# lucidrains/audiolm-pytorch

Hardware: AMD Instinct MI355X
Metric: audio-tokens/sec fwd+bwd, CoarseTransformer d=1024 seq=2048 (higher is better)
Workload: dtype bf16

## Files before the change

audiolm-pytorch_amd/csrc/gemm.hip:

```cpp
#include <algorithm>
#include <cstdlib>
#include <type_traits>

#include "common.hpp"
#include "../../include/audiolm_hip.h"

#ifndef ALM_GEMM_AUX_A
#define ALM_GEMM_AUX_A 0
#endif
#ifndef ALM_GEMM_AUX_B
#define ALM_GEMM_AUX_B 0
#endif

namespace {

constexpr int BK = 64;
constexpr unsigned OOB = 0x80000000u;

typedef __attribute__((address_space(3))) void lds_void;

struct GemmParams {
    const bf16_t* A;
    const bf16_t* B;
    void* C;
// ... 17 lines not shown
    int inl_slices = 0;
};

__device__ __forceinline__ int grouped_tile(int bid, int tiles_m, int tiles_n, int g) {
    const bool rows = g > 0;
    const int ga = rows ? g : -g;
    const int t_in = rows ? tiles_n : tiles_m, t_gr = rows ? tiles_m : tiles_n;
    const int per_group = ga * t_in;
    const int group = bid / per_group, rem = bid % per_group;
    const int first = group * ga;
    const int gsz = min(t_gr - first, ga);
    const int a = first + rem % gsz, b = rem / gsz;
    return rows ? (a | (b << 16)) : (b | (a << 16));
}

template <int BM, int BN, int WM, int WN, int TM, int TNB, bool OUT_F32>
__device__ __forceinline__ void gemm_epilogue(const GemmParams& p, f32x16 (&acc)[TM][TNB], unsigned char* slabs, long long coff0, int m0, int n0,
                                              int wave, int wr, int wc, int lane, int lr, int lh) {
    {
        constexpr int ES = OUT_F32 ? 4 : 2;
        constexpr int WCOLS = 32 * TNB;
        constexpr int ROWB = WCOLS * ES;
        constexpr int NCH = ROWB / 16;
        constexpr int SLAB = 32 * ROWB;
        unsigned char* Cb = reinterpret_cast<unsigned char*>(p.C) + coff0 * ES;
        const bool fast = !p.accumulate && ((p.ldc * ES) & 15) == 0 && ((uintptr_t)Cb & 15) == 0 && (p.N % (16 / ES)) == 0;
        if (fast) {
            unsigned char* slab = slabs + wave * SLAB;
            const int ncol0 = n0 + wc * (BN / WN);
#pragma unroll
            for (int i = 0; i < TM; ++i) {
                const int mrow0 = m0 + wr * (BM / WM) + i * 32;
#pragma unroll
                for (int j = 0; j < TNB; ++j)
#pragma unroll
                    for (int g = 0; g < 4; ++g) {
                        const int c0 = j * 32 + 8 * g + 4 * lh;
                        float v[4];
#pragma unroll
                        for (int c = 0; c < 4; ++c) {
                            v[c] = acc[i][j][4 * g + c] * p.alpha;
                            if (p.bias && ncol0 + c0 + c < p.N) v[c] += p.bias[ncol0 + c0 + c];
                        }
                        if (OUT_F32) {
                            const int ch = c0 / 4;
                            *reinterpret_cast<float4*>(slab + lr * ROWB + ((ch ^ (lr & (NCH - 1))) << 4)) = make_float4(v[0], v[1], v[2], v[3]);
                        } else {
                            const int ch = c0 / 8;
                            *reinterpret_cast<uint2*>(slab + lr * ROWB + ((ch ^ (lr & (NCH - 1))) << 4) + lh * 8) =
                                make_uint2(pack_bf2(v[0], v[1]), pack_bf2(v[2], v[3]));
                        }
                    }
                constexpr int LPR = NCH;
                constexpr int RPI = 64 / LPR;
#pragma unroll
                for (int it = 0; it < 32 / RPI; ++it) {
                    const int row = it * RPI + lane / LPR, ch = lane % LPR;
                    const uint4 val = *reinterpret_cast<const uint4*>(slab + row * ROWB + ((ch ^ (row & (NCH - 1))) << 4));
                    const int gm = mrow0 + row, gn = ncol0 + ch * (16 / ES);
#if defined(ALM_GEMM_WHATIF_NOSTORE)
                    if (gm < p.M && gn < p.N && val.x == 0x7fc12345u) *reinterpret_cast<uint4*>(Cb + ((long long)gm * p.ldc + gn) * ES) = val;
#else
                    if (gm < p.M && gn < p.N) {
                        uint4* dst = reinterpret_cast<uint4*>(Cb + ((long long)gm * p.ldc + gn) * ES);
                        typedef unsigned int u32x4 __attribute__((ext_vector_type(4)));
                        if (p.nt_store) __builtin_nontemporal_store(u32x4{val.x, val.y, val.z, val.w}, reinterpret_cast<u32x4*>(dst)); else *dst = val;
                    }
#endif
                }
            }
            return;
        }
    }
    const long long coff = coff0;
    const bool vec_ok = OUT_F32 ? ((p.ldc & 3) == 0 && (coff & 3) == 0 && ((uintptr_t)p.C & 15) == 0)
                                : ((p.ldc & 3) == 0 && (coff & 3) == 0 && ((uintptr_t)p.C & 7) == 0);
#pragma unroll
    for (int i = 0; i < TM; ++i) {
        const int gm = m0 + wr * (BM / WM) + i * 32 + lr;
        if (gm >= p.M) continue;
#pragma unroll
        for (int j = 0; j < TNB; ++j) {
#pragma unroll
            for (int g = 0; g < 4; ++g) {
                const int gn = n0 + wc * (BN / WN) + j * 32 + 8 * g + 4 * lh;
                if (gn >= p.N) continue;
                float v[4];
#pragma unroll
                for (int c = 0; c < 4; ++c) {
                    v[c] = acc[i][j][4 * g + c] * p.alpha;
                    if (p.bias && gn + c < p.N) v[c] += p.bias[gn + c];
                }
                const long long idx = coff + (long long)gm * p.ldc + gn;
                if (OUT_F32) {
                    float* C = reinterpret_cast<float*>(p.C) + idx;
                    if (vec_ok && gn + 3 < p.N) {
                        float4 o = make_float4(v[0], v[1], v[2], v[3]);
                        if (p.accumulate) { const float4 w = *reinterpret_cast<const float4*>(C); o.x += w.x; o.y += w.y; o.z += w.z; o.w += w.w; }
                        *reinterpret_cast<float4*>(C) = o;
                    } else {
#pragma unroll
                        for (int c = 0; c < 4; ++c)
                            if (gn + c < p.N) C[c] = p.accumulate ? C[c] + v[c] : v[c];
                    }
                } else {
                    bf16_t* C = reinterpret_cast<bf16_t*>(p.C) + idx;
                    if (vec_ok && gn + 3 < p.N) {
                        if (p.accumulate) {
                            const uint2 w = *reinterpret_cast<const uint2*>(C);
                            v[0] += __uint_as_float(w.x << 16); v[1] += __uint_as_float(w.x & 0xffff0000u);
                            v[2] += __uint_as_float(w.y << 16); v[3] += __uint_as_float(w.y & 0xffff0000u);
                        }
                        *reinterpret_cast<uint2*>(C) = make_uint2(pack_bf2(v[0], v[1]), pack_bf2(v[2], v[3]));
                    } else {
#pragma unroll
                        for (int c = 0; c < 4; ++c)
                            if (gn + c < p.N) C[c] = f2bf(p.accumulate ? bf2f(C[c]) + v[c] : v[c]);
                    }
                }
            }
        }
    }
}

template <int N>
__device__ __forceinline__ void wait_vmcnt() {
    static_assert(N == 0 || N == 8 || N == 16, "add the literal");
    if constexpr (N == 0) asm volatile("s_waitcnt vmcnt(0)" ::: "memory");
    else if constexpr (N == 8) asm volatile("s_waitcnt vmcnt(8)" ::: "memory");
    else asm volatile("s_waitcnt vmcnt(16)" ::: "memory");
}

template <int BM, int BN, int WM, int WN, bool TNMODE, bool OUT_F32, int NS = 2>
// ... 197 lines not shown
#pragma unroll 1
        for (int kt = 0; kt < nk; ++kt) {
            const int newer = min(nk - 1 - kt, NS - 2);
            if (newer >= 2) wait_vmcnt<16>(); else if (newer == 1) wait_vmcnt<8>(); else wait_vmcnt<0>();
            asm volatile("s_waitcnt lgkmcnt(0)" ::: "memory");
            __builtin_amdgcn_s_barrier();
            __builtin_amdgcn_sched_barrier(0);
            kstep(smem + ((kt + NS - 1) % NS) * STAGE, smem + (kt % NS) * STAGE, kt);
        }
        __syncthreads();
    }

    constexpr int ES = OUT_F32 ? 4 : 2;
    static_assert(NW * 32 * (32 * TNB * ES) <= 2 * STAGE, "epilogue slab");
    const long long coff0 = z1 * p.sC1 + z2 * p.sC2 + (p.ksplit > 0 ? zs * p.sCk : 0);
    gemm_epilogue<BM, BN, WM, WN, TM, TNB, OUT_F32>(p, acc, smem, coff0, m0, n0, wave, wr, wc, lane, lr, lh);
}

template <int BM, int BN, int WM, int WN, bool TNMODE, bool OUT_F32>
__global__ __launch_bounds__(WM * WN * 64) void gemm_kernel(GemmParams p) {
    gemm_body<BM, BN, WM, WN, TNMODE, OUT_F32>(p, blockIdx.x, blockIdx.y, blockIdx.z);
}

template <int BM, int BN, int WM, int WN, bool TNMODE, bool OUT_F32, int NS>
__global__ __launch_bounds__(WM * WN * 64) void gemm_ring_kernel(GemmParams p) {
    gemm_body<BM, BN, WM, WN, TNMODE, OUT_F32, NS>(p, blockIdx.x, blockIdx.y, blockIdx.z);
}

template <int BM, int BN, int WM, int WN, bool TNMODE, bool OUT_F32>
__global__ __launch_bounds__(WM * WN * 64) void gemm_group2_kernel(GemmParams p0, GemmParams p1, int tiles0) {
    const bool second = (int)blockIdx.x >= tiles0;
    const GemmParams& p = second ? p1 : p0;
    gemm_body<BM, BN, WM, WN, TNMODE, OUT_F32>(p, second ? (int)blockIdx.x - tiles0 : (int)blockIdx.x, 0, 0);
}

#ifdef ALM_GEMM_PROBE
__device__ unsigned long long g_gemm_probe[16384 * 8];
#define GPROBE_DECL unsigned long long pacc[8] = {0, 0, 0, 0, 0, 0, 0, 0}; unsigned long long plast = __builtin_readcyclecounter();
#define GPROBE_T(i) do { __builtin_amdgcn_sched_barrier(0); const unsigned long long pt_ = __builtin_readcyclecounter(); __builtin_amdgcn_sched_barrier(0); pacc[i] += pt_ - plast; plast = pt_; } while (0)
#define GPROBE_FLUSH(slot) do { if (lane == 0 && (slot) < 16384) for (int i_ = 0; i_ < 8; ++i_) g_gemm_probe[(slot) * 8 + i_] = pacc[i_]; } while (0)
#else
#define GPROBE_DECL
#define GPROBE_T(i)
#define GPROBE_FLUSH(slot)
#endif

template <bool TNMODE, bool OUT_F32, bool INL = false>
__device__ __forceinline__ void gemm_stag_body(const GemmParams& p, const int bx, const int by, const int bz) {
    extern __shared__ __attribute__((aligned(1024))) unsigned char smem[];
    GPROBE_DECL
    constexpr int BM = 256, BN = 256, WM = 2, WN = 4, NW = 8, TM = 4, TNB = 2;
    constexpr int AH_BYTES = 128 * BK * 2, B_BYTES = BN * BK * 2;
    constexpr int B_BASE = 4 * AH_BYTES;
    static_assert(B_BASE + 3 * B_BYTES == 163840, "LDS map");

    const int tiles_m = (p.M + BM - 1) / BM, tiles_n = (p.N + BN - 1) / BN;
    int tm, tn, zb, zs;
    if (p.raster >= 1) {
        const int L = bx, xcd = L & 7, j = L >> 3;
        const bool m_major = tiles_m >= tiles_n;
        const int tmaj = m_major ? tiles_m : tiles_n, Q = m_major ? tiles_n : tiles_m;
        const int P = p.plimit > 0 ? p.plimit : tmaj * (p.nbt > 0 ? p.nbt : p.nb2);
// ... 53 lines not shown
#pragma unroll
    for (int j = 0; j < 4; ++j) {
        const int qa = j * 4 + wc;
        const int qb = wr * 16 + j * 4 + wc;
        dstA[j] = (unsigned)(qa * 1024);
        dstB[j] = (unsigned)(qb * 1024);
        if (!TNMODE) {
            const int rowa = wr * 128 + qa * 8 + (lane >> 3), rowb = qb * 8 + (lane >> 3);
            const int ca = (lane & 7) ^ ((rowa >> 1) & 7), cb = (lane & 7) ^ ((rowb >> 1) & 7);
            offA[j] = (unsigned)(rowa * p.lda * 2 + ca * 16);
            offB[j] = (unsigned)(rowb * p.ldb * 2 + cb * 16);
            kcA[j] = ca * 8;
            kcB[j] = cb * 8;
        } else {
            const int st = lane >> 3, kin = (lane >> 1) & 3, half = lane & 1;
            const int ka = qa * 4 + kin, ia = wr * 128 + st * 16 + half * 8;
            const int kgb = qb / 2, partb = qb % 2;
            const int kb = kgb * 4 + kin, ib = partb * 128 + st * 16 + half * 8;
            offA[j] = (unsigned)(ka * p.lda * 2 + ia * 2);
            offB[j] = (unsigned)(kb * p.ldb * 2 + ib * 2);
            kcA[j] = ka;
            kcB[j] = kb;
        }
    }
    const unsigned kstepA = TNMODE ? (unsigned)(BK * p.lda * 2) : (unsigned)(BK * 2);
    const unsigned kstepB = TNMODE ? (unsigned)(BK * p.ldb * 2) : (unsigned)(BK * 2);
    unsigned char* const myA = smem + wr * 2 * AH_BYTES;

    auto stage = [&](int j, unsigned char* ad, unsigned char* bd) {
        const int kleft = Krem - j * BK;
#pragma unroll
        for (int i = 0; i < 4; ++i) {
            const unsigned vo = (kcA[i] < kleft) ? offA[i] : OOB;
            __builtin_amdgcn_raw_ptr_buffer_load_lds(rsA, (lds_void*)(ad + dstA[i]), 16, vo, j * kstepA, 0, ALM_GEMM_AUX_A);
        }
#pragma unroll
        for (int i = 0; i < 4; ++i) {
            const unsigned vo = (kcB[i] < kleft) ? offB[i] : OOB;
            __builtin_amdgcn_raw_ptr_buffer_load_lds(rsB, (lds_void*)(bd + dstB[i]), 16, vo, j * kstepB, 0, ALM_GEMM_AUX_B);
        }
    };

    unsigned fragA[TM], fragB[TNB];
    if (!TNMODE) {
#pragma unroll
        for (int i = 0; i < TM; ++i) fragA[i] = (unsigned)((i * 32 + lr) * 128);
#pragma unroll
        for (int j = 0; j < TNB; ++j) fragB[j] = (unsigned)((wc * 64 + j * 32 + lr) * 128);
    } else {
        const int g = lane >> 4, s = lane & 15;
#pragma unroll
        for (int i = 0; i < TM; ++i) fragA[i] = (unsigned)((((g >> 1) * 2) * 8 + (i * 32) / 16 + (g & 1)) * 128 + s * 8);
#pragma unroll
        for (int j = 0; j < TNB; ++j) fragB[j] = (unsigned)((((g >> 1) * 2) * 16 + (wc * 64 + j * 32) / 16 + (g & 1)) * 128 + s * 8);
    }
    const unsigned sw = (unsigned)((lr >> 1) & 7);

    f32x16 acc[TM][TNB];
#pragma unroll
    for (int i = 0; i < TM; ++i)
#pragma unroll
        for (int j = 0; j < TNB; ++j)
#pragma unroll
            for (int r = 0; r < 16; ++r) acc[i][j][r] = 0.f;

    auto load_frags = [&](const unsigned char* sa, const unsigned char* sb, int ks, bf16x8 (&a)[TM], bf16x8 (&b)[TNB]) {
        if (!TNMODE) {
            const unsigned co = (((unsigned)(ks * 2 + lh)) ^ sw) << 4;
#pragma unroll
            for (int i = 0; i < TM; ++i) a[i] = *reinterpret_cast<const bf16x8*>(sa + fragA[i] + co);
#pragma unroll
            for (int j = 0; j < TNB; ++j) b[j] = *reinterpret_cast<const bf16x8*>(sb + fragB[j] + co);
        } else {
#pragma unroll
            for (int i = 0; i < TM; ++i) {
                const unsigned char* ad = sa + fragA[i] + ks * 4 * 8 * 128;
                a[i] = __builtin_shufflevector(lds_tr16(ad), lds_tr16(ad + 8 * 128), 0, 1, 2, 3, 4, 5, 6, 7);
            }
#pragma unroll
            for (int j = 0; j < TNB; ++j) {
                const unsigned char* bd = sb + fragB[j] + ks * 4 * 16 * 128;
                b[j] = __builtin_shufflevector(lds_tr16(bd), lds_tr16(bd + 16 * 128), 0, 1, 2, 3, 4, 5, 6, 7);
            }
        }
    };
    auto mfma_all = [&](const bf16x8 (&a)[TM], const bf16x8 (&b)[TNB]) {
#pragma unroll
        for (int i = 0; i < TM; ++i)
#pragma unroll
            for (int j = 0; j < TNB; ++j) acc[i][j] = __builtin_amdgcn_mfma_f32_32x32x16_bf16(b[j], a[i], acc[i][j], 0, 0, 0);
    };
    constexpr int NRD = (TNMODE ? 2 : 1) * (TM + TNB);
    auto compute = [&](const unsigned char* sa, const unsigned char* sb) {
        bf16x8 a0[TM], b0[TNB], a1[TM], b1[TNB];
        load_frags(sa, sb, 0, a0, b0);
        load_frags(sa, sb, 1, a1, b1);
        mfma_all(a0, b0);
        load_frags(sa, sb, 2, a0, b0);
        mfma_all(a1, b1);
        load_frags(sa, sb, 3, a1, b1);
        mfma_all(a0, b0);
        mfma_all(a1, b1);
        __builtin_amdgcn_sched_group_barrier(0x100, 2 * NRD, 0);
        for (int g = 0; g < 2; ++g) {
#pragma unroll
            for (int q = 0; q < TM * TNB; ++q) {
                __builtin_amdgcn_sched_group_barrier(0x008, 1, 0);
                if (q < NRD) __builtin_amdgcn_sched_group_barrier(0x100, 1, 0);
            }
            if (NRD > TM * TNB) __builtin_amdgcn_sched_group_barrier(0x100, NRD - TM * TNB, 0);
        }
        __builtin_amdgcn_sched_group_barrier(0x008, 2 * TM * TNB, 0);
    };

    const int nk = (Krem + BK - 1) / BK;
    auto Abuf = [&](int j) { return myA + (j & 1) * AH_BYTES; };
    auto Bbuf = [&](int j) { return smem + B_BASE + (j % 3) * B_BYTES; };
    auto pair = [&](unsigned char* __restrict__ dA, unsigned char* __restrict__ dB, const unsigned char* __restrict__ rA,
                    const unsigned char* __restrict__ rB, int i) {
        if (i < nk) stage(i, dA, dB);
        GPROBE_T(1);
        __builtin_amdgcn_s_barrier();
        GPROBE_T(2);
        if (i >= 1) compute(rA, rB);
        GPROBE_T(3);
        __syncthreads();
        GPROBE_T(4);
    };
    GPROBE_T(0);
    if (wr == 1) __syncthreads();
#pragma unroll 1
    for (int i = 0; i <= nk; ++i) pair(Abuf(i), Bbuf(i), Abuf(i + 1), Bbuf(i + 2), i);
    if (wr == 0) __syncthreads();
    __builtin_amdgcn_s_barrier();

    if constexpr (INL) {
        typedef unsigned int u32x4 __attribute__((ext_vector_type(4)));
        constexpr int SLAB_BYTES = BM * BN * 4, NCHUNK = TM * TNB * 4;
        const int S = p.inl_slices;
        const int tile_lin = zb * (tiles_m * tiles_n) + tm * tiles_n + tn;
        unsigned char* const slab0 = reinterpret_cast<unsigned char*>(p.inl_ws) + (long long)tile_lin * S * SLAB_BYTES;
        {
            const auto rs = __builtin_amdgcn_make_buffer_rsrc(slab0 + (long long)zs * SLAB_BYTES, 0, SLAB_BYTES, 0x00020000);
#pragma unroll
            for (int i = 0; i < TM; ++i)
#pragma unroll
                for (int j = 0; j < TNB; ++j)
#pragma unroll
                    for (int g = 0; g < 4; ++g) {
                        const u32x4 v = {__float_as_uint(acc[i][j][4 * g]), __float_as_uint(acc[i][j][4 * g + 1]), __float_as_uint(acc[i][j][4 * g + 2]),
                                         __float_as_uint(acc[i][j][4 * g + 3])};
                        __builtin_amdgcn_raw_buffer_store_b128(v, rs, t * 16, ((i * TNB + j) * 4 + g) * 8192, 16);
                    }
        }
        asm volatile("s_waitcnt vmcnt(0)" ::: "memory");
        __syncthreads();
        unsigned* const flag = reinterpret_cast<unsigned*>(smem + 163840 - 16);
        if (t == 0) {
            const unsigned old = __hip_atomic_fetch_add(p.inl_cnt + tile_lin, 1u, __ATOMIC_RELAXED, __HIP_MEMORY_SCOPE_AGENT);
            const unsigned last = old == (unsigned)(S - 1);
            if (last) __hip_atomic_store(p.inl_cnt + tile_lin, 0u, __ATOMIC_RELAXED, __HIP_MEMORY_SCOPE_AGENT);
            *flag = last;
        }
        __syncthreads();
        if (*flag == 0) return;
        auto add_slab = [&](int sl, auto first_c) {
            constexpr bool FIRST = decltype(first_c)::value;
            const auto rs = __builtin_amdgcn_make_buffer_rsrc(slab0 + (long long)sl * SLAB_BYTES, 0, SLAB_BYTES, 0x00020000);
#pragma unroll
            for (int cb = 0; cb < NCHUNK; cb += 4) {
                u32x4 v[4];
#pragma unroll
                for (int c = 0; c < 4; ++c) v[c] = __builtin_amdgcn_raw_buffer_load_b128(rs, t * 16, (cb + c) * 8192, 16);
#pragma unroll
                for (int c = 0; c < 4; ++c)
#pragma unroll
                    for (int e = 0; e < 4; ++e) {
                        const int ai = (cb + c) / (4 * TNB), aj = ((cb + c) / 4) % TNB, ar = 4 * ((cb + c) % 4) + e;
                        acc[ai][aj][ar] = FIRST ? __uint_as_float(v[c][e]) : acc[ai][aj][ar] + __uint_as_float(v[c][e]);
                    }
            }
        };
        if (S == 2) {
            add_slab(1 - zs, std::false_type{});
        } else {
            add_slab(0, std::true_type{});
#pragma unroll 1
            for (int sl = 1; sl < S; ++sl) add_slab(sl, std::false_type{});
        }
    }

    const long long coff0 = z1 * p.sC1 + z2 * p.sC2 + (p.ksplit > 0 ? zs * p.sCk : 0);
    GPROBE_T(5);
    gemm_epilogue<BM, BN, WM, WN, TM, TNB, OUT_F32>(p, acc, smem, coff0, m0, n0, wave, wr, wc, lane, lr, lh);
    GPROBE_T(6);
    GPROBE_FLUSH((bx + gridDim.x * (by + gridDim.y * bz)) * 8 + wave);
}


template <bool TNMODE, bool OUT_F32>
__global__ __launch_bounds__(512) void gemm_stag_kernel(GemmParams p) {
    gemm_stag_body<TNMODE, OUT_F32>(p, blockIdx.x, blockIdx.y, blockIdx.z);
}

template <bool OUT_F32>
__global__ __launch_bounds__(512) void gemm_stag_inl_kernel(GemmParams p) {
    gemm_stag_body<false, OUT_F32, true>(p, blockIdx.x, blockIdx.y, blockIdx.z);
}

template <bool TNMODE, bool OUT_F32>
__global__ __launch_bounds__(512) void gemm_stag_group2_kernel(GemmParams p0, GemmParams p1, int tiles0) {
    const bool second = (int)blockIdx.x >= tiles0;
    const GemmParams& p = second ? p1 : p0;
    gemm_stag_body<TNMODE, OUT_F32>(p, second ? (int)blockIdx.x - tiles0 : (int)blockIdx.x, 0, 0);
}

template <bool TNMODE, bool OUT_F32>
__global__ __launch_bounds__(256) void gemm_w4_kernel(GemmParams p) {
    extern __shared__ __attribute__((aligned(1024))) unsigned char smem[];
    GPROBE_DECL
    constexpr int BM = 256, BN = 256, WM = 2, WN = 2, NW = 4, TM = 4, TNB = 4;
    constexpr int A_BYTES = BM * BK * 2, B_BYTES = BN * BK * 2, STAGE = A_BYTES + B_BYTES;
    constexpr int NIA = BM / 8 / NW, NIB = BN / 8 / NW;
    static_assert(NIA + NIB == 16, "the counted waits below assume 16 pieces per wave and stage");

    const int tiles_m = (p.M + BM - 1) / BM, tiles_n = (p.N + BN - 1) / BN;
    int tm, tn, zb, zs;
    if (p.raster >= 1) {
        const int L = blockIdx.x, xcd = L & 7, j = L >> 3;
// ... 214 lines not shown
        __builtin_amdgcn_sched_barrier(0);
        GPROBE_T(4);
    };
    using T = std::true_type;
    using F = std::false_type;
    int kt = 0;
#pragma unroll 1
    for (; kt + 2 < nk; ++kt) kstep(smem + (kt & 1) * STAGE, smem + ((kt & 1) ^ 1) * STAGE, kt, T{}, T{});
    if (kt + 1 < nk) { kstep(smem + (kt & 1) * STAGE, smem + ((kt & 1) ^ 1) * STAGE, kt, F{}, T{}); ++kt; }
    kstep(smem + (kt & 1) * STAGE, smem + ((kt & 1) ^ 1) * STAGE, kt, F{}, F{});
    __syncthreads();

    constexpr int ES = OUT_F32 ? 4 : 2;
    static_assert(NW * 32 * (32 * TNB * ES) <= 2 * STAGE, "epilogue slab");
    const long long coff0 = z1 * p.sC1 + z2 * p.sC2 + (p.ksplit > 0 ? zs * p.sCk : 0);
    gemm_epilogue<BM, BN, WM, WN, TM, TNB, OUT_F32>(p, acc, smem, coff0, m0, n0, wave, wr, wc, lane, lr, lh);
    GPROBE_T(6);
    GPROBE_FLUSH((blockIdx.x + gridDim.x * (blockIdx.y + gridDim.y * blockIdx.z)) * 4 + wave);
}

__global__ __launch_bounds__(256) void splitk_reduce_kernel(const float* __restrict__ ws, int splits, long long mn, long long slice_stride, int N,
                                                            float* __restrict__ C, long long ldc, long long sC, int accumulate,
                                                            int nb2 = 0x40000000, long long sC1 = 0) {
    ws += (long long)blockIdx.y * mn;
    C += (long long)(blockIdx.y / nb2) * sC1 + (long long)(blockIdx.y % nb2) * sC;
    const bool vec = (N & 3) == 0 && (ldc & 3) == 0 && ((uintptr_t)C & 15) == 0 && (mn & 3) == 0 && (slice_stride & 3) == 0;
    if (vec) {
        const long long mn4 = mn >> 2;
        for (long long i = (long long)blockIdx.x * 256 + threadIdx.x; i < mn4; i += (long long)gridDim.x * 256) {
            float4 s = make_float4(0.f, 0.f, 0.f, 0.f);
            for (int z = 0; z < splits; ++z) {
// ... 218 lines not shown

template <bool OUT_F32>
int launch_ring(const GemmParams& p, int ny, int nz, hipStream_t st) {
    constexpr int smem = 4 * (128 + 128) * BK * 2;
    static bool attr_done = false;
    auto kfn = gemm_ring_kernel<128, 128, 2, 2, false, OUT_F32, 4>;
    if (!attr_done) {
        hipError_t e = hipFuncSetAttribute(reinterpret_cast<const void*>(kfn), hipFuncAttributeMaxDynamicSharedMemorySize, smem);
        if (e != hipSuccess) return (int)e;
        attr_done = true;
    }
    hipLaunchKernelGGL(kfn, dim3(((p.M + 127) / 128) * ((p.N + 127) / 128), ny, nz), dim3(256), smem, st, p);
    return 0;
}

template <bool TNMODE, bool OUT_F32>
int launch_stag(const GemmParams& p, int ny, int nz, hipStream_t st) {
    constexpr int smem = 163840;
    static bool attr_done = false;
    auto kfn = gemm_stag_kernel<TNMODE, OUT_F32>;
    if (!attr_done) {
        hipError_t e = hipFuncSetAttribute(reinterpret_cast<const void*>(kfn), hipFuncAttributeMaxDynamicSharedMemorySize, smem);
        if (e != hipSuccess) return (int)e;
        attr_done = true;
    }
    const int tiles_m = (p.M + 255) / 256, tiles_n = (p.N + 255) / 256;
    if (p.raster >= 1) {
        const int tmaj = tiles_m >= tiles_n ? tiles_m : tiles_n, Q = tiles_m >= tiles_n ? tiles_n : tiles_m;
        const int PL = ((p.plimit > 0 ? p.plimit : tmaj * ny) + 7) / 8;
        hipLaunchKernelGGL(kfn, dim3(8 * PL * Q * nz), dim3(512), smem, st, p);
        return 0;
    }
    hipLaunchKernelGGL(kfn, dim3(tiles_m * tiles_n, ny, nz), dim3(512), smem, st, p);
    return 0;
}


template <bool OUT_F32>
int launch_stag_inl(const GemmParams& p, int ny, hipStream_t st) {
    constexpr int smem = 163840;
    static bool attr_done = false;
    auto kfn = gemm_stag_inl_kernel<OUT_F32>;
    if (!attr_done) {
        hipError_t e = hipFuncSetAttribute(reinterpret_cast<const void*>(kfn), hipFuncAttributeMaxDynamicSharedMemorySize, smem);
        if (e != hipSuccess) return (int)e;
        attr_done = true;
    }
    const int tiles_m = (p.M + 255) / 256, tiles_n = (p.N + 255) / 256;
    hipLaunchKernelGGL(kfn, dim3(tiles_m * tiles_n, ny, p.inl_slices), dim3(512), smem, st, p);
    return 0;
}

template <bool TNMODE, bool OUT_F32>
int launch_w4(const GemmParams& p, int ny, int nz, hipStream_t st) {
    constexpr int smem = 131072;
    static bool attr_done = false;
    auto kfn = gemm_w4_kernel<TNMODE, OUT_F32>;
// ... 41 lines not shown
template <bool TNMODE>
int launch_gemm(const GemmParams& p0, int ny, int nz, int out_f32, int tile, hipStream_t st, bool hook = true, bool only256 = false) {
    static const int big_tile = [] { const char* e = getenv("ALM_GEMM_BIG_TILE"); return e ? atoi(e) : 0; }();
    static const int nt_store = [] { const char* e = getenv("ALM_GEMM_NT_STORE"); return e ? atoi(e) : 0; }();
    GemmParams p = p0;
    int tl = pick_tile(p.M, p.N, ny * nz, tile, TNMODE);
    if (tl < 0) return ALM_ERR_UNSUPPORTED;
    p.group_m = pick_group(p, tl);
    p.nt_store = (nt_store == 1 || (nt_store == 2 && !out_f32)) ? 1 : 0;
    if (hook && tl != 1 && (big_tile == 2 || big_tile == 13 || big_tile == 14 || (big_tile == 11 && !only256))) tl = big_tile;
    static const int w4_mink = [] { const char* e = getenv("ALM_GEMM_W4_MINK"); return e ? atoi(e) : 0; }();
    if (hook && w4_mink > 0 && tl == 13 && tile == 0 && (p.ksplit > 0 ? p.ksplit : p.K) >= w4_mink) tl = 14;
    static const int w4_tn_mink = [] { const char* e = getenv("ALM_GEMM_W4_TN_MINK"); return e ? atoi(e) : 8192; }();
    if (TNMODE && hook && w4_tn_mink > 0 && tl == 13 && (p.ksplit > 0 ? p.ksplit : p.K) >= w4_tn_mink) tl = 14;
    if (tl == 14) return out_f32 ? launch_w4<TNMODE, true>(p, ny, nz, st) : launch_w4<TNMODE, false>(p, ny, nz, st);
    if (tl == 13) return out_f32 ? launch_stag<TNMODE, true>(p, ny, nz, st) : launch_stag<TNMODE, false>(p, ny, nz, st);
    static const int mid_tile = [] { const char* e = getenv("ALM_GEMM_MID_TILE"); return e ? atoi(e) : 0; }();
    if (!TNMODE && hook && mid_tile && tl == 1 && tile == 0 && p.ksplit == 0 && p.M >= 256 && p.N >= 512 &&
        (long long)((p.M + 255) / 256) * ((p.N + 127) / 128) * ny >= 192) tl = 15;
    static const int ring_on = [] { const char* e = getenv("ALM_GEMM_RING"); return e ? atoi(e) : 1; }();
    if (!TNMODE && hook && ring_on && tl == 1 && tile == 0 && p.ksplit == 0 && p.raster == 0 && p.K >= 256 &&
        (long long)((p.M + 127) / 128) * ((p.N + 127) / 128) * ny * nz <= 256) tl = 16;
    if (tl == 16) { if (TNMODE || p.raster != 0) return ALM_ERR_UNSUPPORTED; return out_f32 ? launch_ring<true>(p, ny, nz, st) : launch_ring<false>(p, ny, nz, st); }
    if (tl == 15) return out_f32 ? launch_cfg<256, 128, 4, 2, TNMODE, true>(p, ny, nz, st) : launch_cfg<256, 128, 4, 2, TNMODE, false>(p, ny, nz, st);
    if (tl == 11) return out_f32 ? launch_cfg<384, 256, 2, 4, TNMODE, true>(p, ny, nz, st) : launch_cfg<384, 256, 2, 4, TNMODE, false>(p, ny, nz, st);
    if (tl == 17) { if (TNMODE) return ALM_ERR_UNSUPPORTED; return out_f32 ? launch_cfg<320, 256, 2, 4, false, true>(p, ny, nz, st) : launch_cfg<320, 256, 2, 4, false, false>(p, ny, nz, st); }
    if (tl == 2) return out_f32 ? launch_cfg<256, 256, 2, 4, TNMODE, true>(p, ny, nz, st) : launch_cfg<256, 256, 2, 4, TNMODE, false>(p, ny, nz, st);
    return out_f32 ? launch_cfg<128, 128, 2, 2, TNMODE, true>(p, ny, nz, st) : launch_cfg<128, 128, 2, 2, TNMODE, false>(p, ny, nz, st);
}

bool view_too_big(long long rows, long long ld) { return rows * ld * 2 >= 0x7fffffffLL; }
// ... 35 lines not shown
    if (pl.slices == 1) return launch_gemm<false>(p0, ny, 1, out_f32, 13, st, false);
    const long long need = INL_CNT_BYTES + tiles * pl.slices * INL_SLAB_BYTES;
    if (!ws || ws_bytes < need || ((uintptr_t)ws & 15)) {
        if (force_slices > 0) return ALM_ERR_BAD_ARG;
        return launch_gemm<false>(p0, ny, 1, out_f32, 0, st);
    }
    GemmParams p = p0;
    const int ksteps = (p.K + BK - 1) / BK;
    p.ksplit = (ksteps + pl.slices - 1) / pl.slices * BK;
    p.sCk = 0;
    p.inl_slices = (p.K + p.ksplit - 1) / p.ksplit;
    if (p.inl_slices < 2) return launch_gemm<false>(p0, ny, 1, out_f32, 13, st, false);
    p.inl_cnt = reinterpret_cast<unsigned*>(ws);
    p.inl_ws = reinterpret_cast<float*>(reinterpret_cast<unsigned char*>(ws) + INL_CNT_BYTES);
    p.group_m = pick_group(p, 13);
    return out_f32 ? launch_stag_inl<true>(p, ny, st) : launch_stag_inl<false>(p, ny, st);
}

struct SplitPlan { int tile, slices; };

int pick_raster(int M, int N, int nb, int tile) {
    const int bm = tile >= 2 ? 256 : 128;
    const int tmm = (M + bm - 1) / bm, tnn = (N + bm - 1) / bm;
    const int P = (tmm >= tnn ? tmm : tnn) * nb;
    return (P % 8 == 0 || P >= 20) ? 1 : 0;
}
SplitPlan splitk_plan(int M, int N, int K, int nb) {
    SplitPlan best{1, 1};
    double best_t = 1e30;
    for (int tile = 1; tile <= 2; ++tile) {
        if (tile == 2 && (M < 256 || N < 256)) continue;
// ... 131 lines not shown
        const long long a = (long long)((M0 + 255) / 256) * ((N0 + 255) / 256), b = (long long)((M1 + 255) / 256) * ((N1 + 255) / 256);
        if (a + b >= 192 && a + b <= 256 && (a & 7) == 0) t0 = t1 = 13;
    }
    const int bm = t0 == 1 ? 128 : 256;
    const int tiles0 = ((M0 + bm - 1) / bm) * ((N0 + bm - 1) / bm), tiles1 = ((M1 + bm - 1) / bm) * ((N1 + bm - 1) / bm);
    if (!on || t0 != t1 || (t0 != 1 && t0 != 13) || (tiles0 & 7)) {
        int rc = alm_gemm_bf16_nt(A0, B0, C0, nullptr, M0, N0, K0, lda0, ldb0, ldc0, 1, 1, 0, 0, 0, 0, 0, 0, 1.f, out_f32, 0, stream);
        if (rc) return rc;
        return alm_gemm_bf16_nt(A1, B1, C1, nullptr, M1, N1, K1, lda1, ldb1, ldc1, 1, 1, 0, 0, 0, 0, 0, 0, 1.f, out_f32, 0, stream);
    }
    GemmParams p0{(const bf16_t*)A0, (const bf16_t*)B0, C0, nullptr, M0, N0, K0, lda0, ldb0, ldc0, 1, 0, 0, 0, 0, 0, 0, 1.f, 0, 0, 0, 0, 1};
    GemmParams p1{(const bf16_t*)A1, (const bf16_t*)B1, C1, nullptr, M1, N1, K1, lda1, ldb1, ldc1, 1, 0, 0, 0, 0, 0, 0, 1.f, 0, 0, 0, 0, 1};
    p0.group_m = pick_group(p0, t0);
    p1.group_m = pick_group(p1, t1);
    auto launch = [&](auto kfn, int which, int threads, int smem) -> int {
        static bool attr_done[4] = {false, false, false, false};
        if (!attr_done[which]) {
            hipError_t e = hipFuncSetAttribute(reinterpret_cast<const void*>(kfn), hipFuncAttributeMaxDynamicSharedMemorySize, smem);
            if (e != hipSuccess) return (int)e;
            attr_done[which] = true;
        }
        hipLaunchKernelGGL(kfn, dim3(tiles0 + tiles1), dim3(threads), smem, st, p0, p1, tiles0);
        return 0;
    };
    int rc;
    if (t0 == 1) rc = out_f32 ? launch(gemm_group2_kernel<128, 128, 2, 2, false, true>, 0, 256, 2 * (128 + 128) * BK * 2)
                              : launch(gemm_group2_kernel<128, 128, 2, 2, false, false>, 1, 256, 2 * (128 + 128) * BK * 2);
    else rc = out_f32 ? launch(gemm_stag_group2_kernel<false, true>, 2, 512, 163840) : launch(gemm_stag_group2_kernel<false, false>, 3, 512, 163840);
    if (rc) return rc;
    ALM_LAUNCH_CHECK();
    return 0;
}

extern "C" int alm_gemm_bf16_nt_tile(const void* A, const void* B, void* C, const float* bias, int M, int N, int K, long long lda,
                                     long long ldb, long long ldc, float alpha, int out_f32, int accumulate, int tile, void* stream) {
    if (M <= 0 || N <= 0) return 0;
    if (K <= 0 || (K & 7) || (lda & 7) || (ldb & 7) || ((uintptr_t)A & 15) || ((uintptr_t)B & 15)) return ALM_ERR_BAD_ARG;
    if (view_too_big(384, lda) || view_too_big(256, ldb)) return ALM_ERR_UNSUPPORTED;
    GemmParams p{(const bf16_t*)A, (const bf16_t*)B, C, bias, M, N, K, lda, ldb, ldc, 1, 0, 0, 0, 0, 0, 0, alpha, accumulate, 0, 0, 0, 1};
    int rc = launch_gemm<false>(p, 1, 1, out_f32, tile, (hipStream_t)stream, false);
    if (rc) return rc;
    ALM_LAUNCH_CHECK();
    return 0;
// ... 234 lines not shown
```

Before: 1.438 million.

## Use 16x16x32 MFMA in staggered 256-tile GEMM kernel by default

Adds an MF16 variant of the staggered 256x256 GEMM body that computes with 16x16x32 bf16 MFMA instructions instead of 32x32x16. This changes the fragment addressing, LDS swizzle and accumulator layout, and generalises the epilogue and inline split-K reduction to both accumulator shapes. The variant is on by default through an environment switch. The aim is a better MFMA issue and LDS-read interleaving schedule. The trade-off is more LDS fragment reads per MFMA and a riskier scheduling pattern.

```diff
diff --git a/audiolm-pytorch_amd/csrc/gemm.hip b/audiolm-pytorch_amd/csrc/gemm.hip
--- a/audiolm-pytorch_amd/csrc/gemm.hip
+++ b/audiolm-pytorch_amd/csrc/gemm.hip
@@ -55,9 +55,26 @@
     return rows ? (a | (b << 16)) : (b | (a << 16));
 }
 
-template <int BM, int BN, int WM, int WN, int TM, int TNB, bool OUT_F32>
-__device__ __forceinline__ void gemm_epilogue(const GemmParams& p, f32x16 (&acc)[TM][TNB], unsigned char* slabs, long long coff0, int m0, int n0,
-                                              int wave, int wr, int wc, int lane, int lr, int lh) {
+template <int TNB, typename AccV, int AM, int AN>
+__device__ __forceinline__ void acc_quad(AccV (&acc)[AM][AN], int i, int q, int lane, int& r, int& c0, float (&v)[4]) {
+    if constexpr (std::is_same<AccV, f32x16>::value) {
+        const int j = q / 4, g = q % 4;
+        r = lane & 31;
+        c0 = j * 32 + 8 * g + 4 * (lane >> 5);
+#pragma unroll
+        for (int c = 0; c < 4; ++c) v[c] = acc[i][j][4 * g + c];
+    } else {
+        const int h = q / (2 * TNB), j = q % (2 * TNB);
+        r = h * 16 + (lane & 15);
+        c0 = j * 16 + 4 * (lane >> 4);
+#pragma unroll
+        for (int c = 0; c < 4; ++c) v[c] = acc[2 * i + h][j][c];
+    }
+}
+
+template <int BM, int BN, int WM, int WN, int TM, int TNB, bool OUT_F32, typename AccV, int AM, int AN>
+__device__ __forceinline__ void gemm_epilogue(const GemmParams& p, AccV (&acc)[AM][AN], unsigned char* slabs, long long coff0, int m0, int n0,
+                                              int wave, int wr, int wc, int lane) {
     {
         constexpr int ES = OUT_F32 ? 4 : 2;
         constexpr int WCOLS = 32 * TNB;
@@ -73,25 +90,24 @@
             for (int i = 0; i < TM; ++i) {
                 const int mrow0 = m0 + wr * (BM / WM) + i * 32;
 #pragma unroll
-                for (int j = 0; j < TNB; ++j)
-#pragma unroll
-                    for (int g = 0; g < 4; ++g) {
-                        const int c0 = j * 32 + 8 * g + 4 * lh;
-                        float v[4];
-#pragma unroll
-                        for (int c = 0; c < 4; ++c) {
-                            v[c] = acc[i][j][4 * g + c] * p.alpha;
-                            if (p.bias && ncol0 + c0 + c < p.N) v[c] += p.bias[ncol0 + c0 + c];
-                        }
-                        if (OUT_F32) {
-                            const int ch = c0 / 4;
-                            *reinterpret_cast<float4*>(slab + lr * ROWB + ((ch ^ (lr & (NCH - 1))) << 4)) = make_float4(v[0], v[1], v[2], v[3]);
-                        } else {
-                            const int ch = c0 / 8;
-                            *reinterpret_cast<uint2*>(slab + lr * ROWB + ((ch ^ (lr & (NCH - 1))) << 4) + lh * 8) =
-                                make_uint2(pack_bf2(v[0], v[1]), pack_bf2(v[2], v[3]));
-                        }
+                for (int q = 0; q < 4 * TNB; ++q) {
+                    int r, c0;
+                    float v[4];
+                    acc_quad<TNB>(acc, i, q, lane, r, c0, v);
+#pragma unroll
+                    for (int c = 0; c < 4; ++c) {
+                        v[c] *= p.alpha;
+                        if (p.bias && ncol0 + c0 + c < p.N) v[c] += p.bias[ncol0 + c0 + c];
                     }
+                    if (OUT_F32) {
+                        const int ch = c0 / 4;
+                        *reinterpret_cast<float4*>(slab + r * ROWB + ((ch ^ (r & (NCH - 1))) << 4)) = make_float4(v[0], v[1], v[2], v[3]);
+                    } else {
+                        const int ch = c0 / 8;
+                        *reinterpret_cast<uint2*>(slab + r * ROWB + ((ch ^ (r & (NCH - 1))) << 4) + ((c0 >> 2) & 1) * 8) =
+                            make_uint2(pack_bf2(v[0], v[1]), pack_bf2(v[2], v[3]));
+                    }
+                }
                 constexpr int LPR = NCH;
                 constexpr int RPI = 64 / LPR;
 #pragma unroll
@@ -118,46 +134,44 @@
                                 : ((p.ldc & 3) == 0 && (coff & 3) == 0 && ((uintptr_t)p.C & 7) == 0);
 #pragma unroll
     for (int i = 0; i < TM; ++i) {
-        const int gm = m0 + wr * (BM / WM) + i * 32 + lr;
-        if (gm >= p.M) continue;
-#pragma unroll
-        for (int j = 0; j < TNB; ++j) {
-#pragma unroll
-            for (int g = 0; g < 4; ++g) {
-                const int gn = n0 + wc * (BN / WN) + j * 32 + 8 * g + 4 * lh;
-                if (gn >= p.N) continue;
-                float v[4];
-#pragma unroll
-                for (int c = 0; c < 4; ++c) {
-                    v[c] = acc[i][j][4 * g + c] * p.alpha;
-                    if (p.bias && gn + c < p.N) v[c] += p.bias[gn + c];
+#pragma unroll
+        for (int q = 0; q < 4 * TNB; ++q) {
+            int r, c0;
+            float v[4];
+            acc_quad<TNB>(acc, i, q, lane, r, c0, v);
+            const int gm = m0 + wr * (BM / WM) + i * 32 + r;
+            const int gn = n0 + wc * (BN / WN) + c0;
+            if (gm >= p.M || gn >= p.N) continue;
+#pragma unroll
+            for (int c = 0; c < 4; ++c) {
+                v[c] *= p.alpha;
+                if (p.bias && gn + c < p.N) v[c] += p.bias[gn + c];
+            }
+            const long long idx = coff + (long long)gm * p.ldc + gn;
+            if (OUT_F32) {
+                float* C = reinterpret_cast<float*>(p.C) + idx;
+                if (vec_ok && gn + 3 < p.N) {
+                    float4 o = make_float4(v[0], v[1], v[2], v[3]);
+                    if (p.accumulate) { const float4 w = *reinterpret_cast<const float4*>(C); o.x += w.x; o.y += w.y; o.z += w.z; o.w += w.w; }
+                    *reinterpret_cast<float4*>(C) = o;
+                } else {
+#pragma unroll
+                    for (int c = 0; c < 4; ++c)
+                        if (gn + c < p.N) C[c] = p.accumulate ? C[c] + v[c] : v[c];
                 }
-                const long long idx = coff + (long long)gm * p.ldc + gn;
-                if (OUT_F32) {
-                    float* C = reinterpret_cast<float*>(p.C) + idx;
-                    if (vec_ok && gn + 3 < p.N) {
-                        float4 o = make_float4(v[0], v[1], v[2], v[3]);
-                        if (p.accumulate) { const float4 w = *reinterpret_cast<const float4*>(C); o.x += w.x; o.y += w.y; o.z += w.z; o.w += w.w; }
-                        *reinterpret_cast<float4*>(C) = o;
-                    } else {
-#pragma unroll
-                        for (int c = 0; c < 4; ++c)
-                            if (gn + c < p.N) C[c] = p.accumulate ? C[c] + v[c] : v[c];
+            } else {
+                bf16_t* C = reinterpret_cast<bf16_t*>(p.C) + idx;
+                if (vec_ok && gn + 3 < p.N) {
+                    if (p.accumulate) {
+                        const uint2 w = *reinterpret_cast<const uint2*>(C);
+                        v[0] += __uint_as_float(w.x << 16); v[1] += __uint_as_float(w.x & 0xffff0000u);
+                        v[2] += __uint_as_float(w.y << 16); v[3] += __uint_as_float(w.y & 0xffff0000u);
                     }
+                    *reinterpret_cast<uint2*>(C) = make_uint2(pack_bf2(v[0], v[1]), pack_bf2(v[2], v[3]));
                 } else {
-                    bf16_t* C = reinterpret_cast<bf16_t*>(p.C) + idx;
-                    if (vec_ok && gn + 3 < p.N) {
-                        if (p.accumulate) {
-                            const uint2 w = *reinterpret_cast<const uint2*>(C);
-                            v[0] += __uint_as_float(w.x << 16); v[1] += __uint_as_float(w.x & 0xffff0000u);
-                            v[2] += __uint_as_float(w.y << 16); v[3] += __uint_as_float(w.y & 0xffff0000u);
-                        }
-                        *reinterpret_cast<uint2*>(C) = make_uint2(pack_bf2(v[0], v[1]), pack_bf2(v[2], v[3]));
-                    } else {
-#pragma unroll
-                        for (int c = 0; c < 4; ++c)
-                            if (gn + c < p.N) C[c] = f2bf(p.accumulate ? bf2f(C[c]) + v[c] : v[c]);
-                    }
+#pragma unroll
+                    for (int c = 0; c < 4; ++c)
+                        if (gn + c < p.N) C[c] = f2bf(p.accumulate ? bf2f(C[c]) + v[c] : v[c]);
                 }
             }
         }
@@ -385,7 +399,7 @@
     constexpr int ES = OUT_F32 ? 4 : 2;
     static_assert(NW * 32 * (32 * TNB * ES) <= 2 * STAGE, "epilogue slab");
     const long long coff0 = z1 * p.sC1 + z2 * p.sC2 + (p.ksplit > 0 ? zs * p.sCk : 0);
-    gemm_epilogue<BM, BN, WM, WN, TM, TNB, OUT_F32>(p, acc, smem, coff0, m0, n0, wave, wr, wc, lane, lr, lh);
+    gemm_epilogue<BM, BN, WM, WN, TM, TNB, OUT_F32>(p, acc, smem, coff0, m0, n0, wave, wr, wc, lane);
 }
 
 template <int BM, int BN, int WM, int WN, bool TNMODE, bool OUT_F32>
@@ -416,7 +430,7 @@
 #define GPROBE_FLUSH(slot)
 #endif
 
-template <bool TNMODE, bool OUT_F32, bool INL = false>
+template <bool TNMODE, bool OUT_F32, bool INL = false, bool MF16 = false>
 __device__ __forceinline__ void gemm_stag_body(const GemmParams& p, const int bx, const int by, const int bz) {
     extern __shared__ __attribute__((aligned(1024))) unsigned char smem[];
     GPROBE_DECL
@@ -500,9 +514,10 @@
             kcB[j] = cb * 8;
         } else {
             const int st = lane >> 3, kin = (lane >> 1) & 3, half = lane & 1;
-            const int ka = qa * 4 + kin, ia = wr * 128 + st * 16 + half * 8;
+            const int xa = MF16 ? (qa >> 1) & 1 : 0, xb = MF16 ? (qb >> 2) & 1 : 0;
+            const int ka = qa * 4 + kin, ia = wr * 128 + (st ^ xa) * 16 + half * 8;
             const int kgb = qb / 2, partb = qb % 2;
-            const int kb = kgb * 4 + kin, ib = partb * 128 + st * 16 + half * 8;
+            const int kb = kgb * 4 + kin, ib = partb * 128 + (st ^ xb) * 16 + half * 8;
             offA[j] = (unsigned)(ka * p.lda * 2 + ia * 2);
             offB[j] = (unsigned)(kb * p.ldb * 2 + ib * 2);
             kcA[j] = ka;
@@ -527,8 +542,16 @@
         }
     };
 
-    unsigned fragA[TM], fragB[TNB];
-    if (!TNMODE) {
+    constexpr int FA = MF16 ? 2 * TM : TM, FB = MF16 ? 2 * TNB : TNB;
+    unsigned fragA[FA], fragB[FB];
+    if (MF16) {
+        const int g = lane >> 4, s = lane & 15;
+#pragma unroll
+        for (int i = 0; i < FA; ++i) fragA[i] = TNMODE ? (unsigned)(((2 * g) * 8 + (i ^ (g & 1))) * 128 + s * 8) : (unsigned)((i * 16 + s) * 128);
+#pragma unroll
+        for (int j = 0; j < FB; ++j)
+            fragB[j] = TNMODE ? (unsigned)(((2 * g) * 16 + ((wc * 4 + j) ^ (g & 1))) * 128 + s * 8) : (unsigned)((wc * 64 + j * 16 + s) * 128);
+    } else if (!TNMODE) {
 #pragma unroll
         for (int i = 0; i < TM; ++i) fragA[i] = (unsigned)((i * 32 + lr) * 128);
 #pragma unroll
@@ -540,15 +563,17 @@
 #pragma unroll
         for (int j = 0; j < TNB; ++j) fragB[j] = (unsigned)((((g >> 1) * 2) * 16 + (wc * 64 + j * 32) / 16 + (g & 1)) * 128 + s * 8);
     }
-    const unsigned sw = (unsigned)((lr >> 1) & 7);
-
-    f32x16 acc[TM][TNB];
-#pragma unroll
-    for (int i = 0; i < TM; ++i)
-#pragma unroll
-        for (int j = 0; j < TNB; ++j)
-#pragma unroll
-            for (int r = 0; r < 16; ++r) acc[i][j][r] = 0.f;
+    const unsigned sw = MF16 ? (unsigned)(((lane & 15) >> 1) & 7) : (unsigned)((lr >> 1) & 7);
+
+    using AccV = typename std::conditional<MF16, f32x4, f32x16>::type;
+    constexpr int AREG = MF16 ? 4 : 16;
+    AccV acc[FA][FB];
+#pragma unroll
+    for (int i = 0; i < FA; ++i)
+#pragma unroll
+        for (int j = 0; j < FB; ++j)
+#pragma unroll
+            for (int r = 0; r < AREG; ++r) acc[i][j][r] = 0.f;
 
     auto load_frags = [&](const unsigned char* sa, const unsigned char* sb, int ks, bf16x8 (&a)[TM], bf16x8 (&b)[TNB]) {
         if (!TNMODE) {
@@ -571,10 +596,12 @@
         }
     };
     auto mfma_all = [&](const bf16x8 (&a)[TM], const bf16x8 (&b)[TNB]) {
-#pragma unroll
-        for (int i = 0; i < TM; ++i)
-#pragma unroll
-            for (int j = 0; j < TNB; ++j) acc[i][j] = __builtin_amdgcn_mfma_f32_32x32x16_bf16(b[j], a[i], acc[i][j], 0, 0, 0);
+        if constexpr (!MF16) {
+#pragma unroll
+            for (int i = 0; i < TM; ++i)
+#pragma unroll
+                for (int j = 0; j < TNB; ++j) acc[i][j] = __builtin_amdgcn_mfma_f32_32x32x16_bf16(b[j], a[i], acc[i][j], 0, 0, 0);
+        }
     };
     constexpr int NRD = (TNMODE ? 2 : 1) * (TM + TNB);
     auto compute = [&](const unsigned char* sa, const unsigned char* sb) {
@@ -598,6 +625,51 @@
         }
         __builtin_amdgcn_sched_group_barrier(0x008, 2 * TM * TNB, 0);
     };
+    auto load_frags16 = [&](const unsigned char* sa, const unsigned char* sb, int ks, bf16x8 (&a)[FA], bf16x8 (&b)[FB]) {
+        if (!TNMODE) {
+            const unsigned co = (((unsigned)(ks * 4 + (lane >> 4))) ^ sw) << 4;
+#pragma unroll
+            for (int i = 0; i < FA; ++i) a[i] = *reinterpret_cast<const bf16x8*>(sa + fragA[i] + co);
+#pragma unroll
+            for (int j = 0; j < FB; ++j) b[j] = *reinterpret_cast<const bf16x8*>(sb + fragB[j] + co);
+        } else {
+#pragma unroll
+            for (int i = 0; i < FA; ++i) {
+                const unsigned char* ad = sa + fragA[i] + ks * 8 * 8 * 128;
+                a[i] = __builtin_shufflevector(lds_tr16(ad), lds_tr16(ad + 8 * 128), 0, 1, 2, 3, 4, 5, 6, 7);
+            }
+#pragma unroll
+            for (int j = 0; j < FB; ++j) {
+                const unsigned char* bd = sb + fragB[j] + ks * 8 * 16 * 128;
+                b[j] = __builtin_shufflevector(lds_tr16(bd), lds_tr16(bd + 16 * 128), 0, 1, 2, 3, 4, 5, 6, 7);
+            }
+        }
+    };
+    auto mfma_all16 = [&](const bf16x8 (&a)[FA], const bf16x8 (&b)[FB]) {
+        if constexpr (MF16) {
+#pragma unroll
+            for (int i = 0; i < FA; ++i)
+#pragma unroll
+                for (int j = 0; j < FB; ++j) acc[i][j] = __builtin_amdgcn_mfma_f32_16x16x32_bf16(b[j], a[i], acc[i][j], 0, 0, 0);
+        }
+    };
+    constexpr int NRD16 = (TNMODE ? 2 : 1) * (FA + FB);
+    constexpr int NMF16 = FA * FB;
+    static_assert(!MF16 || NRD16 <= NMF16, "at most one read per MFMA gap");
+    auto compute16 = [&](const unsigned char* sa, const unsigned char* sb) {
+        bf16x8 a0[FA], b0[FB], a1[FA], b1[FB];
+        load_frags16(sa, sb, 0, a0, b0);
+        load_frags16(sa, sb, 1, a1, b1);
+        mfma_all16(a0, b0);
+        mfma_all16(a1, b1);
+        __builtin_amdgcn_sched_group_barrier(0x100, NRD16, 0);
+#pragma unroll
+        for (int q = 0; q < NMF16; ++q) {
+            __builtin_amdgcn_sched_group_barrier(0x008, 1, 0);
+            if ((q + 1) * NRD16 / NMF16 > q * NRD16 / NMF16) __builtin_amdgcn_sched_group_barrier(0x100, 1, 0);
+        }
+        __builtin_amdgcn_sched_group_barrier(0x008, NMF16, 0);
+    };
 
     const int nk = (Krem + BK - 1) / BK;
     auto Abuf = [&](int j) { return myA + (j & 1) * AH_BYTES; };
@@ -608,7 +680,9 @@
         GPROBE_T(1);
         __builtin_amdgcn_s_barrier();
         GPROBE_T(2);
-        if (i >= 1) compute(rA, rB);
+        if (i >= 1) {
+            if constexpr (MF16) compute16(rA, rB); else compute(rA, rB);
+        }
         GPROBE_T(3);
         __syncthreads();
         GPROBE_T(4);
@@ -623,21 +697,24 @@
     if constexpr (INL) {
         typedef unsigned int u32x4 __attribute__((ext_vector_type(4)));
         constexpr int SLAB_BYTES = BM * BN * 4, NCHUNK = TM * TNB * 4;
+        auto accr = [&](int c, int e) -> float {
+            if constexpr (MF16) return acc[c / FB][c % FB][e];
+            else return acc[c / (4 * TNB)][(c / 4) % TNB][4 * (c % 4) + e];
+        };
+        auto accw = [&](int c, int e, float v) {
+            if constexpr (MF16) acc[c / FB][c % FB][e] = v;
+            else acc[c / (4 * TNB)][(c / 4) % TNB][4 * (c % 4) + e] = v;
+        };
         const int S = p.inl_slices;
         const int tile_lin = zb * (tiles_m * tiles_n) + tm * tiles_n + tn;
         unsigned char* const slab0 = reinterpret_cast<unsigned char*>(p.inl_ws) + (long long)tile_lin * S * SLAB_BYTES;
         {
             const auto rs = __builtin_amdgcn_make_buffer_rsrc(slab0 + (long long)zs * SLAB_BYTES, 0, SLAB_BYTES, 0x00020000);
 #pragma unroll
-            for (int i = 0; i < TM; ++i)
-#pragma unroll
-                for (int j = 0; j < TNB; ++j)
-#pragma unroll
-                    for (int g = 0; g < 4; ++g) {
-                        const u32x4 v = {__float_as_uint(acc[i][j][4 * g]), __float_as_uint(acc[i][j][4 * g + 1]), __float_as_uint(acc[i][j][4 * g + 2]),
-                                         __float_as_uint(acc[i][j][4 * g + 3])};
-                        __builtin_amdgcn_raw_buffer_store_b128(v, rs, t * 16, ((i * TNB + j) * 4 + g) * 8192, 16);
-                    }
+            for (int c = 0; c < NCHUNK; ++c) {
+                const u32x4 v = {__float_as_uint(accr(c, 0)), __float_as_uint(accr(c, 1)), __float_as_uint(accr(c, 2)), __float_as_uint(accr(c, 3))};
+                __builtin_amdgcn_raw_buffer_store_b128(v, rs, t * 16, c * 8192, 16);
+            }
         }
         asm volatile("s_waitcnt vmcnt(0)" ::: "memory");
         __syncthreads();
@@ -661,10 +738,7 @@
 #pragma unroll
                 for (int c = 0; c < 4; ++c)
 #pragma unroll
-                    for (int e = 0; e < 4; ++e) {
-                        const int ai = (cb + c) / (4 * TNB), aj = ((cb + c) / 4) % TNB, ar = 4 * ((cb + c) % 4) + e;
-                        acc[ai][aj][ar] = FIRST ? __uint_as_float(v[c][e]) : acc[ai][aj][ar] + __uint_as_float(v[c][e]);
-                    }
+                    for (int e = 0; e < 4; ++e) accw(cb + c, e, FIRST ? __uint_as_float(v[c][e]) : accr(cb + c, e) + __uint_as_float(v[c][e]));
             }
         };
         if (S == 2) {
@@ -678,27 +752,27 @@
 
     const long long coff0 = z1 * p.sC1 + z2 * p.sC2 + (p.ksplit > 0 ? zs * p.sCk : 0);
     GPROBE_T(5);
-    gemm_epilogue<BM, BN, WM, WN, TM, TNB, OUT_F32>(p, acc, smem, coff0, m0, n0, wave, wr, wc, lane, lr, lh);
+    gemm_epilogue<BM, BN, WM, WN, TM, TNB, OUT_F32>(p, acc, smem, coff0, m0, n0, wave, wr, wc, lane);
     GPROBE_T(6);
     GPROBE_FLUSH((bx + gridDim.x * (by + gridDim.y * bz)) * 8 + wave);
 }
 
 
-template <bool TNMODE, bool OUT_F32>
+template <bool TNMODE, bool OUT_F32, bool MF16>
 __global__ __launch_bounds__(512) void gemm_stag_kernel(GemmParams p) {
-    gemm_stag_body<TNMODE, OUT_F32>(p, blockIdx.x, blockIdx.y, blockIdx.z);
-}
-
-template <bool OUT_F32>
+    gemm_stag_body<TNMODE, OUT_F32, false, MF16>(p, blockIdx.x, blockIdx.y, blockIdx.z);
+}
+
+template <bool OUT_F32, bool MF16>
 __global__ __launch_bounds__(512) void gemm_stag_inl_kernel(GemmParams p) {
-    gemm_stag_body<false, OUT_F32, true>(p, blockIdx.x, blockIdx.y, blockIdx.z);
-}
-
-template <bool TNMODE, bool OUT_F32>
+    gemm_stag_body<false, OUT_F32, true, MF16>(p, blockIdx.x, blockIdx.y, blockIdx.z);
+}
+
+template <bool TNMODE, bool OUT_F32, bool MF16>
 __global__ __launch_bounds__(512) void gemm_stag_group2_kernel(GemmParams p0, GemmParams p1, int tiles0) {
     const bool second = (int)blockIdx.x >= tiles0;
     const GemmParams& p = second ? p1 : p0;
-    gemm_stag_body<TNMODE, OUT_F32>(p, second ? (int)blockIdx.x - tiles0 : (int)blockIdx.x, 0, 0);
+    gemm_stag_body<TNMODE, OUT_F32, false, MF16>(p, second ? (int)blockIdx.x - tiles0 : (int)blockIdx.x, 0, 0);
 }
 
 template <bool TNMODE, bool OUT_F32>
@@ -943,7 +1017,7 @@
     constexpr int ES = OUT_F32 ? 4 : 2;
     static_assert(NW * 32 * (32 * TNB * ES) <= 2 * STAGE, "epilogue slab");
     const long long coff0 = z1 * p.sC1 + z2 * p.sC2 + (p.ksplit > 0 ? zs * p.sCk : 0);
-    gemm_epilogue<BM, BN, WM, WN, TM, TNB, OUT_F32>(p, acc, smem, coff0, m0, n0, wave, wr, wc, lane, lr, lh);
+    gemm_epilogue<BM, BN, WM, WN, TM, TNB, OUT_F32>(p, acc, smem, coff0, m0, n0, wave, wr, wc, lane);
     GPROBE_T(6);
     GPROBE_FLUSH((blockIdx.x + gridDim.x * (blockIdx.y + gridDim.y * blockIdx.z)) * 4 + wave);
 }
@@ -1192,11 +1266,19 @@
     return 0;
 }
 
-template <bool TNMODE, bool OUT_F32>
+#ifndef ALM_GEMM_MFMA_DEFAULT
+#define ALM_GEMM_MFMA_DEFAULT 16
+#endif
+bool stag_mf16() {
+    static const int v = [] { const char* e = getenv("ALM_GEMM_MFMA"); return e ? atoi(e) : ALM_GEMM_MFMA_DEFAULT; }();
+    return v == 16;
+}
+
+template <bool TNMODE, bool OUT_F32, bool MF16>
 int launch_stag(const GemmParams& p, int ny, int nz, hipStream_t st) {
     constexpr int smem = 163840;
     static bool attr_done = false;
-    auto kfn = gemm_stag_kernel<TNMODE, OUT_F32>;
+    auto kfn = gemm_stag_kernel<TNMODE, OUT_F32, MF16>;
     if (!attr_done) {
         hipError_t e = hipFuncSetAttribute(reinterpret_cast<const void*>(kfn), hipFuncAttributeMaxDynamicSharedMemorySize, smem);
         if (e != hipSuccess) return (int)e;
@@ -1214,11 +1296,11 @@
 }
 
 
-template <bool OUT_F32>
+template <bool OUT_F32, bool MF16>
 int launch_stag_inl(const GemmParams& p, int ny, hipStream_t st) {
     constexpr int smem = 163840;
     static bool attr_done = false;
-    auto kfn = gemm_stag_inl_kernel<OUT_F32>;
+    auto kfn = gemm_stag_inl_kernel<OUT_F32, MF16>;
     if (!attr_done) {
         hipError_t e = hipFuncSetAttribute(reinterpret_cast<const void*>(kfn), hipFuncAttributeMaxDynamicSharedMemorySize, smem);
         if (e != hipSuccess) return (int)e;
@@ -1290,7 +1372,10 @@
     static const int w4_tn_mink = [] { const char* e = getenv("ALM_GEMM_W4_TN_MINK"); return e ? atoi(e) : 8192; }();
     if (TNMODE && hook && w4_tn_mink > 0 && tl == 13 && (p.ksplit > 0 ? p.ksplit : p.K) >= w4_tn_mink) tl = 14;
     if (tl == 14) return out_f32 ? launch_w4<TNMODE, true>(p, ny, nz, st) : launch_w4<TNMODE, false>(p, ny, nz, st);
-    if (tl == 13) return out_f32 ? launch_stag<TNMODE, true>(p, ny, nz, st) : launch_stag<TNMODE, false>(p, ny, nz, st);
+    if (tl == 13) {
+        if (stag_mf16()) return out_f32 ? launch_stag<TNMODE, true, true>(p, ny, nz, st) : launch_stag<TNMODE, false, true>(p, ny, nz, st);
+        return out_f32 ? launch_stag<TNMODE, true, false>(p, ny, nz, st) : launch_stag<TNMODE, false, false>(p, ny, nz, st);
+    }
     static const int mid_tile = [] { const char* e = getenv("ALM_GEMM_MID_TILE"); return e ? atoi(e) : 0; }();
     if (!TNMODE && hook && mid_tile && tl == 1 && tile == 0 && p.ksplit == 0 && p.M >= 256 && p.N >= 512 &&
         (long long)((p.M + 255) / 256) * ((p.N + 127) / 128) * ny >= 192) tl = 15;
@@ -1356,7 +1441,8 @@
     p.inl_cnt = reinterpret_cast<unsigned*>(ws);
     p.inl_ws = reinterpret_cast<float*>(reinterpret_cast<unsigned char*>(ws) + INL_CNT_BYTES);
     p.group_m = pick_group(p, 13);
-    return out_f32 ? launch_stag_inl<true>(p, ny, st) : launch_stag_inl<false>(p, ny, st);
+    if (stag_mf16()) return out_f32 ? launch_stag_inl<true, true>(p, ny, st) : launch_stag_inl<false, true>(p, ny, st);
+    return out_f32 ? launch_stag_inl<true, false>(p, ny, st) : launch_stag_inl<false, false>(p, ny, st);
 }
 
 struct SplitPlan { int tile, slices; };
@@ -1518,7 +1604,7 @@
     p0.group_m = pick_group(p0, t0);
     p1.group_m = pick_group(p1, t1);
     auto launch = [&](auto kfn, int which, int threads, int smem) -> int {
-        static bool attr_done[4] = {false, false, false, false};
+        static bool attr_done[6] = {false, false, false, false, false, false};
         if (!attr_done[which]) {
             hipError_t e = hipFuncSetAttribute(reinterpret_cast<const void*>(kfn), hipFuncAttributeMaxDynamicSharedMemorySize, smem);
             if (e != hipSuccess) return (int)e;
@@ -1530,7 +1616,8 @@
     int rc;
     if (t0 == 1) rc = out_f32 ? launch(gemm_group2_kernel<128, 128, 2, 2, false, true>, 0, 256, 2 * (128 + 128) * BK * 2)
                               : launch(gemm_group2_kernel<128, 128, 2, 2, false, false>, 1, 256, 2 * (128 + 128) * BK * 2);
-    else rc = out_f32 ? launch(gemm_stag_group2_kernel<false, true>, 2, 512, 163840) : launch(gemm_stag_group2_kernel<false, false>, 3, 512, 163840);
+    else if (stag_mf16()) rc = out_f32 ? launch(gemm_stag_group2_kernel<false, true, true>, 4, 512, 163840) : launch(gemm_stag_group2_kernel<false, false, true>, 5, 512, 163840);
+    else rc = out_f32 ? launch(gemm_stag_group2_kernel<false, true, false>, 2, 512, 163840) : launch(gemm_stag_group2_kernel<false, false, false>, 3, 512, 163840);
     if (rc) return rc;
     ALM_LAUNCH_CHECK();
     return 0;
```

New measurement: 1.457 million, median of 6. +1.3%, better.
